# jdidion/atropos

Measured on AMD Instinct MI355X. Metric: reads/s (whole node) 150 bp SE adapter-align, higher is better.
Workload: dtype int32

## Files before the change

atropos_amd/csrc/filter_kernels.hip:

```cpp
#define ATR_DEFINE_FILTER_KERNELS
#include "locate_fast.hpp"
#include "side_stream.hpp"

namespace atr {

constexpr long long FAST_SERIAL_READS = 65536;
constexpr long long FAST_SERIAL_READS_LINKED = 64;

window_launcher window_group_0(int), window_group_1(int), window_group_2(int), window_group_3(int);

static BandParams band_params(const atr_aligner *a) {
    BandParams bp;
    memset(&bp, 0, sizeof(bp));
    for (int i = 0; i < a->p.m && i < FILTER_MAX_M; ++i) bp.rrep[i] = (uint32_t)(a->codes[i] & 15u) * 0x11111111u;
    bp.and_mode = (a->wildcard_ref || a->wildcard_query) ? 1 : 0;
    bp.noindel = a->indel_cost > a->p.k ? 1 : 0;
    return bp;
}

int launch_linked_band(const void *d_wave, int nad, bool and_mode, const uint4 *packed, const int32_t *lens, long long nreads,
                       int nchunks, int max_len, const uint4 *front, uint4 *out, FastWork wk, hipStream_t st);

static LinkedArgs no_linked_args() {
    LinkedArgs la;
    memset(&la, 0, sizeof(la));
    return la;
}

typedef window_launcher (*window_group_fn)(int);
static const window_group_fn window_groups[4] = {window_group_0, window_group_1, window_group_2, window_group_3};

void launch_fast_scan(FastWork wk, hipStream_t st) {
    hipLaunchKernelGGL(scan_bins_kernel, dim3((wk.nused + SCAN_CHUNK - 1) / SCAN_CHUNK, wk.nbins / 256), dim3(256), 0, st, wk);
    hipLaunchKernelGGL(scan_total_kernel, dim3(1), dim3(1024), 0, st, wk);
}

constexpr int DP_STREAMS = 4;
int launch_fast_dp(const atr_aligner *a, const uint4 *packed, const int32_t *lens, long long nreads, int nchunks,
                   int max_len, uint4 *out, FastWork wk, const LinkedArgs *la, int idx, int count, hipStream_t st, bool planes,
                   bool one_stream) {
    static thread_local SideStream side[DP_STREAMS];
    if (planes && la) return (int)hipErrorInvalidValue;
    if (count < 1 || count > DP_STREAMS || idx < 0 || idx >= count) return (int)hipErrorInvalidValue;
    hipError_t e = hipSuccess;
    const bool serial = one_stream || nreads <= (count == 1 ? FAST_SERIAL_READS : FAST_SERIAL_READS_LINKED);
    if (serial) {
        const BandParams bp = band_params(a);
        const dim3 bgrid((unsigned)std::max<long long>(1, std::min<long long>((nreads + 3) / 4, 4096)));
        const LinkedArgs none = la ? *la : no_linked_args();
        if (la) {
            if (bp.and_mode) hipLaunchKernelGGL((band_kernel<true, true>), bgrid, dim3(256), 0, st, a->p, bp, packed, lens, nreads, nchunks, max_len, out, wk, none);
            else             hipLaunchKernelGGL((band_kernel<false, true>), bgrid, dim3(256), 0, st, a->p, bp, packed, lens, nreads, nchunks, max_len, out, wk, none);
        } else if (planes) {
            if (bp.and_mode) hipLaunchKernelGGL((band_kernel<true, false, true>), bgrid, dim3(256), 0, st, a->p, bp, packed, lens, nreads, nchunks, max_len, out, wk, none);
            else             hipLaunchKernelGGL((band_kernel<false, false, true>), bgrid, dim3(256), 0, st, a->p, bp, packed, lens, nreads, nchunks, max_len, out, wk, none);
        } else {
            if (bp.and_mode) hipLaunchKernelGGL((band_kernel<true, false>), bgrid, dim3(256), 0, st, a->p, bp, packed, lens, nreads, nchunks, max_len, out, wk, none);
            else             hipLaunchKernelGGL((band_kernel<false, false>), bgrid, dim3(256), 0, st, a->p, bp, packed, lens, nreads, nchunks, max_len, out, wk, none);
        }
        e = hipGetLastError();
        if (e != hipSuccess) return (int)e;
        const int mts = round_up_rows(a->p.m) / ROW_GRAN - 1;
        return window_groups[mts / 4](mts % 4)(a, packed, lens, nreads, nchunks, max_len, out, wk, la, st, planes);
    }
    const int nside = (la && la->win_count != 1) ? 1 : std::min(count, 3);
    hipStream_t bst = st;
    if (idx == 0) {
        static const bool urgent = [] { const char *x = getenv("ATR_WINDOW_PRIORITY"); return !(x && x[0] == '0'); }();
        for (int k = 0; k < nside; ++k) if (!side[k].ready(urgent)) return (int)hipErrorInvalidValue;
        e = hipEventRecord(side[0].fork, st);
        for (int k = 0; k < nside && e == hipSuccess; ++k) e = hipStreamWaitEvent(side[k].stream, side[0].fork, 0);
        if (e != hipSuccess) return (int)e;
    }
    const dim3 block(256);
    {
        const BandParams bp = band_params(a);
        const dim3 bgrid((unsigned)std::min<long long>((nreads + 255) / 256, 4096));
        if (la && la->multi) {
            if (idx == 0) {
                const int rc = launch_linked_band(la->multi, count, la->multi_and, packed, lens, nreads, nchunks, max_len, la->front,
                                                  out, wk, bst);
                if (rc != 0) return rc;
            }
        } else if (la) {
            if (bp.and_mode) hipLaunchKernelGGL((band_kernel<true, true>), bgrid, block, 0, bst, a->p, bp, packed, lens, nreads, nchunks, max_len, out, wk, *la);
            else             hipLaunchKernelGGL((band_kernel<false, true>), bgrid, block, 0, bst, a->p, bp, packed, lens, nreads, nchunks, max_len, out, wk, *la);
        } else if (planes) {
            const LinkedArgs none = no_linked_args();
            if (bp.and_mode) hipLaunchKernelGGL((band_kernel<true, false, true>), bgrid, block, 0, bst, a->p, bp, packed, lens, nreads, nchunks, max_len, out, wk, none);
            else             hipLaunchKernelGGL((band_kernel<false, false, true>), bgrid, block, 0, bst, a->p, bp, packed, lens, nreads, nchunks, max_len, out, wk, none);
        } else {
            const LinkedArgs none = no_linked_args();
            if (bp.and_mode) hipLaunchKernelGGL((band_kernel<true, false>), bgrid, block, 0, bst, a->p, bp, packed, lens, nreads, nchunks, max_len, out, wk, none);
            else             hipLaunchKernelGGL((band_kernel<false, false>), bgrid, block, 0, bst, a->p, bp, packed, lens, nreads, nchunks, max_len, out, wk, none);
        }
    }
    e = hipGetLastError();
    if (e != hipSuccess) return (int)e;
    const int mt = round_up_rows(a->p.m) / ROW_GRAN - 1;
    const int rc = window_groups[mt / 4](mt % 4)(a, packed, lens, nreads, nchunks, max_len, out, wk, la,
                                                 side[idx % nside].stream, planes);
    if (rc != 0) return rc;
    if (idx == count - 1) {
        for (int k = 0; k < nside && e == hipSuccess; ++k) {
            e = hipEventRecord(side[k].join, side[k].stream);
            if (e == hipSuccess) e = hipStreamWaitEvent(st, side[k].join, 0);
        }
    }
    return (int)e;
}

int launch_locate_fast(const atr_aligner *a, const uint4 *packed, const int32_t *lens, long long nreads,
                       int nchunks, int max_len, uint4 *out, void *work, hipStream_t st) {
    FastWork wk = fast_carve(work, nreads);
    wk.nused = fast_blocks_for((nreads + 63) / 64);
    wk.lpw = nreads <= 8192 ? 0 : 64;
    const FilterParams &fp = aligner_filter_params(a);
    const bool wide = fp.rows > 32, ragged = lens != nullptr;
    const dim3 grid(wk.nused), block(256);
    if (wide) {
        if (ragged) hipLaunchKernelGGL((filter_kernel<true, true>), grid, block, 0, st, a->p, fp, packed, lens, nreads, nchunks, max_len, out, wk);
        else        hipLaunchKernelGGL((filter_kernel<true, false>), grid, block, 0, st, a->p, fp, packed, lens, nreads, nchunks, max_len, out, wk);
    } else {
        if (ragged) hipLaunchKernelGGL((filter_kernel<false, true>), grid, block, 0, st, a->p, fp, packed, lens, nreads, nchunks, max_len, out, wk);
        else        hipLaunchKernelGGL((filter_kernel<false, false>), grid, block, 0, st, a->p, fp, packed, lens, nreads, nchunks, max_len, out, wk);
    }
    launch_fast_scan(wk, st);
    hipLaunchKernelGGL(scatter_kernel, dim3(wk.nused), dim3(256), 0, st, nreads, a->p.m,
                       (!ragged || !(a->flags & ATR_START_WITHIN_SEQ1)) ? 1 : 0, wk);
    return launch_fast_dp(a, packed, lens, nreads, nchunks, max_len, out, wk, nullptr, 0, 1, st, false, false);
}

int launch_prefix_band(const atr_aligner *a, const uint4 *packed, const int32_t *lens, long long nreads, int nchunks,
                       int max_len, uint4 *out, hipStream_t st) {
    const BandParams bp = band_params(a);
    const dim3 grid((unsigned)((nreads + 255) / 256)), block(256);
    if (bp.and_mode) hipLaunchKernelGGL((prefix_band_kernel<true>), grid, block, 0, st, a->p, bp, packed, lens, nreads, nchunks, max_len, out);
    else             hipLaunchKernelGGL((prefix_band_kernel<false>), grid, block, 0, st, a->p, bp, packed, lens, nreads, nchunks, max_len, out);
    return (int)hipGetLastError();
}

}
```

atropos_amd/csrc/locate_fast.hpp:

```cpp
#ifndef ATR_LOCATE_FAST_HPP
#define ATR_LOCATE_FAST_HPP

#include <algorithm>
#include "locate_kernel.hpp"
#include "filter_core.hpp"
#include "linked_core.hpp"
#include "piece_core.hpp"
#include "fast_work.hpp"

namespace atr {
inline const FilterParams &aligner_filter_params(const atr_aligner *a) {
    struct Slot { unsigned long long uid = 0; FilterParams fp; };
    static thread_local Slot slots[4];
    static thread_local unsigned turn = 0;
    if (a->uid != 0)
        for (Slot &s : slots) if (s.uid == a->uid) return s.fp;
    Slot &s = slots[turn++ & 3u];
    s.fp = filter_params(a->peq, a->codes, a->p.m, a->flags, a->wildcard_ref || a->wildcard_query, a->p.thr, a->p.min_overlap);
    s.uid = a->uid;
    return s.fp;
}
inline const FilterParams &aligner_piece_filter_params(const atr_aligner *a) {
    struct Slot { unsigned long long uid = 0; FilterParams fp; };
    static thread_local Slot slots[4];
    static thread_local unsigned turn = 0;
    if (a->uid != 0)
        for (Slot &s : slots) if (s.uid == a->uid) return s.fp;
    Slot &s = slots[turn++ & 3u];
    s.fp = filter_params(a->peq, a->codes, a->p.m, a->flags, a->wildcard_ref || a->wildcard_query, a->p.thr, a->p.min_overlap, true);
    s.uid = a->uid;
    return s.fp;
}
}

namespace atr {

struct LinkedArgs {
    int bin0;
    const uint4 *front;
    LinkedPost post;
    const void *multi;
    bool multi_and;
    const LocateParams *multi_p;
    const LinkedPost *multi_post;
    int a0, win_count;
};

inline int fast_blocks_for(long long ntiles) {
    return (int)std::max<long long>(1, std::min<long long>(FAST_BLOCKS, (ntiles + 3) / 4));
}

__device__ __forceinline__ int dp_lanes_per_wave(long long tasks, long long grid_waves, int fixed) {
    if (fixed) return fixed;
    int lpw = 1;
    while (lpw < 64 && (long long)lpw * grid_waves < tasks) lpw <<= 1;
    return lpw;
}

constexpr int SCAN_CHUNK = 64, SCAN_CHUNKS = FAST_BLOCKS / SCAN_CHUNK;
static_assert(FAST_BLOCKS % SCAN_CHUNK == 0 && SCAN_CHUNKS % 16 == 0 && SCAN_CHUNK % 16 == 0, "scan kernels walk 16 rows at a time");
__device__ __forceinline__ uint32_t fast_slot0(const FastWork &wk, int bin) {
    return wk.binbase[bin] + wk.chunks[(size_t)(blockIdx.x / SCAN_CHUNK) * wk.nbins + bin] +
           wk.counts[(size_t)blockIdx.x * wk.nbins + bin];
}

#ifdef ATR_DEFINE_FILTER_KERNELS
template <bool WIDE, bool RAGGED>
__global__ __launch_bounds__(256) void filter_kernel(const LocateParams p, const FilterParams fp,
                                                     const uint4 *__restrict__ packed,
                                                     const int32_t *__restrict__ lens, long long nreads, int nchunks,
                                                     int max_len, uint4 *__restrict__ out, FastWork wk) {
    __shared__ uint2 s_peq[16];
    __shared__ uint32_t s_hist[FILTER_BINS];
    const Uniform u = make_uniform(p, round_up_rows_dev(p.m));
    if (threadIdx.x < 16) s_peq[threadIdx.x] = make_uint2((uint32_t)fp.peq[threadIdx.x], (uint32_t)(fp.peq[threadIdx.x] >> 32));
    if (threadIdx.x < FILTER_BINS) s_hist[threadIdx.x] = 0;
    __syncthreads();

    const int lane = threadIdx.x & 63, wave = __builtin_amdgcn_readfirstlane((int)(threadIdx.x >> 6));
    const long long ntiles = (nreads + 63) >> 6;
    long long t0, t1;
    block_tiles(ntiles, t0, t1, wk.nused);
    for (long long tile = t0 + wave; tile < t1; tile += 4) {
        const long long r = tile * 64 + lane;
        const bool live = r < nreads;
        const int n = live ? (RAGGED ? lens[r] : max_len) : 0;
        FilterState F;
        filter_init(F, u, fp.rows);
        const int jhi = RAGGED ? wave_max_i32(n) : max_len;
        const int jfull = RAGGED ? wave_min_i32(live ? n : 0x7fffffff) : max_len;
        const uint4 *tp = packed + (size_t)tile * nchunks * 64 + lane;
        if (jhi > 0) {
            const int c1 = (jhi + 31) >> 5;
            uint4 nxt = tp[0];
            uint2 ea[8], eb[8];
            auto fetch_masks = [&](uint32_t w, uint2 (&e)[8]) { fetch_peq8(s_peq, w, e); };
            const uint32_t kreg = (uint32_t)u.k;
            fetch_masks(nxt.x, ea);
            for (int c = 0; c < c1; ++c) {
                uint4 cur = nxt;
                if (c + 1 < c1) nxt = tp[(size_t)(c + 1) * 64];
                int j = c * 32;
#pragma unroll
                for (int d = 0; d < 4; ++d) {
                    uint2 (&e)[8] = (d & 1) ? eb : ea;
                    fetch_masks(d == 0 ? cur.y : d == 1 ? cur.z : d == 2 ? cur.w : nxt.x, (d & 1) ? ea : eb);
                    if (j + 8 <= (RAGGED ? jfull : jhi)) {
#pragma unroll
                        for (int b = 0; b < 8; ++b) filter_step<WIDE>(F, e[b].x, e[b].y, kreg);
                        j += 8;
                    } else {
#pragma unroll
                        for (int b = 0; b < 8; ++b) {
                            ++j;
                            if (j <= jhi && (!RAGGED || j <= n)) filter_step<WIDE>(F, e[b].x, e[b].y, kreg);
                        }
                    }
                    if (j >= jhi) break;
                }
                filter_fold(F, RAGGED ? min(n, min(j, jhi)) : min(j, jhi), fp.rows, kreg);
            }
        }
        uint32_t ww_lane = 0u;
        if (live) {
            uint32_t rec[4];
            const uint32_t ww = filter_decide<WIDE>(F, u, fp, (const uint32_t *)tp, nchunks, n, rec);
            ww_lane = ww;
            if (!window_valid(ww)) out[r] = make_uint4(rec[0], rec[1], rec[2], rec[3]);
            else atomicAdd(&s_hist[window_bin(ww, u.m, !RAGGED || ragged_rows_bins(u.sr))], 1u);
        }
        const uint64_t um = __ballot(window_valid(ww_lane));
        if (lane == 0) wk.mask[tile] = um;
        if (window_valid(ww_lane)) wk.win[tile * 64 + __popcll(um & ((1ull << lane) - 1ull))] = ww_lane;
    }
    __syncthreads();
    if (threadIdx.x < FILTER_BINS) wk.counts[(size_t)blockIdx.x * FILTER_BINS + threadIdx.x] = s_hist[threadIdx.x];
}

__global__ __launch_bounds__(256) void scan_bins_kernel(FastWork wk) {
    const int bin = blockIdx.y * 256 + threadIdx.x;
    uint32_t *col = wk.counts + (size_t)blockIdx.x * SCAN_CHUNK * wk.nbins + bin;
    const int rows = min(SCAN_CHUNK, wk.nused - (int)blockIdx.x * SCAN_CHUNK);
    uint32_t run = 0;
    for (int b0 = 0; b0 < rows; b0 += 16) {
        uint32_t v[16];
#pragma unroll
        for (int i = 0; i < 16; ++i) v[i] = b0 + i < rows ? col[(size_t)(b0 + i) * wk.nbins] : 0u;
#pragma unroll
        for (int i = 0; i < 16; ++i) { if (b0 + i < rows) col[(size_t)(b0 + i) * wk.nbins] = run; run += v[i]; }
    }
    wk.chunks[(size_t)blockIdx.x * wk.nbins + bin] = run;
}

__global__ __launch_bounds__(1024) void scan_total_kernel(FastWork wk) {
    __shared__ uint32_t s_part[1024];
    const int b = threadIdx.x;
    uint32_t mine = 0u;
    if (b < wk.nbins) {
        uint32_t *col = wk.chunks + b;
        const int chunks = (wk.nused + SCAN_CHUNK - 1) / SCAN_CHUNK;
        for (int c0 = 0; c0 < chunks; c0 += 16) {
            uint32_t v[16];
#pragma unroll
            for (int i = 0; i < 16; ++i) v[i] = c0 + i < chunks ? col[(size_t)(c0 + i) * wk.nbins] : 0u;
#pragma unroll
            for (int i = 0; i < 16; ++i) { if (c0 + i < chunks) col[(size_t)(c0 + i) * wk.nbins] = mine; mine += v[i]; }
        }
    }
    s_part[b] = mine;
    __syncthreads();
    for (int off = 1; off < 1024; off <<= 1) {
        const uint32_t add = b >= off ? s_part[b - off] : 0u;
        __syncthreads();
        s_part[b] += add;
        __syncthreads();
    }
    if (b < wk.nbins) wk.binbase[b] = s_part[b] - mine;
    if (b == 1023) { wk.binbase[wk.nbins] = s_part[1023]; wk.total[0] = s_part[1023]; }
}

__global__ __launch_bounds__(256) void scatter_kernel(long long nreads, int m, int by_rows, FastWork wk) {
    __shared__ uint32_t s_cur[FILTER_BINS];
    if (threadIdx.x < FILTER_BINS)
        s_cur[threadIdx.x] = fast_slot0(wk, threadIdx.x);
    __syncthreads();
    const long long ntiles = (nreads + 63) >> 6;
    long long t0, t1;
    block_tiles(ntiles, t0, t1, wk.nused);
    constexpr int SCATTER_ROUNDS = 4;
    const long long rend = min(nreads, t1 * 64);
    for (long long r0 = t0 * 64 + threadIdx.x; r0 < rend; r0 += 256 * SCATTER_ROUNDS) {
        uint64_t um[SCATTER_ROUNDS];
        uint32_t ww[SCATTER_ROUNDS];
#pragma unroll
        for (int t = 0; t < SCATTER_ROUNDS; ++t) {
            const long long r = r0 + 256 * t;
            um[t] = r < rend ? wk.mask[r >> 6] : 0ull;
        }
#pragma unroll
        for (int t = 0; t < SCATTER_ROUNDS; ++t) {
            const long long r = r0 + 256 * t;
            const int lane = (int)(r & 63);
            ww[t] = ((um[t] >> lane) & 1ull) ? wk.win[(r & ~63ll) + __popcll(um[t] & ((1ull << lane) - 1ull))] : 0u;
        }
#pragma unroll
        for (int t = 0; t < SCATTER_ROUNDS; ++t) {
            const long long r = r0 + 256 * t;
            if (window_valid(ww[t]))
                wk.order[atomicAdd(&s_cur[window_bin(ww[t], m, by_rows != 0)], 1u)] = make_uint2((uint32_t)r, ww[t]);
        }
    }
}
template <bool AND_MODE, bool LINKED, bool PLANES = false>
__global__ __launch_bounds__(256) void band_kernel(const LocateParams p, const BandParams bp,
                                                   const uint4 *__restrict__ packed, const int32_t *__restrict__ lens,
                                                   long long nreads, int nchunks, int max_len, uint4 *__restrict__ out,
                                                   FastWork wk, const LinkedArgs la) {
    __shared__ int16_t s_thr[ATR_MAX_REF_LEN + 2];
    __shared__ uint32_t s_stream[4][BAND_STREAM][64];
    __shared__ uint32_t s_spread_flat[PLANES ? 1024 : 1];
    uint32_t (*s_spread)[256] = (uint32_t (*)[256])s_spread_flat;
    const Uniform u = make_uniform(p, round_up_rows_dev(p.m));
    for (int i = threadIdx.x; i <= u.m + 1; i += 256) s_thr[i] = p.thr[i];
    if constexpr (PLANES) piece_spread_fill(s_spread);
    __syncthreads();
    const long long base = LINKED ? (long long)wk.binbase[la.bin0] : 0;
    const long long total = (long long)wk.binbase[(LINKED ? la.bin0 : 0) + BAND_BINS];
    const int lane = threadIdx.x & 63;
    const int lpw = dp_lanes_per_wave(total - base, (long long)gridDim.x * 4, wk.lpw);
    const long long nwaves = (total - base + lpw - 1) / lpw;
    for (long long wv = (long long)blockIdx.x * 4 + __builtin_amdgcn_readfirstlane((int)(threadIdx.x >> 6)); wv < nwaves;
         wv += (long long)gridDim.x * 4) {
        const long long slot = base + wv * lpw + lane;
        const bool live = lane < lpw && slot < total;
        const uint2 task = live ? wk.order[slot] : make_uint2(0u, 0u);
        const long long r = (long long)task.x;
        const uint32_t ww = task.y;
        const int n = live ? (lens ? lens[r] : max_len) : 0;
        const bool last = live && window_scan(ww);
        const bool any_last = wave_max_i32(last ? 1 : 0) != 0, any_rowm = wave_max_i32(live && !last ? 1 : 0) != 0;
        const int s_lane = (live && !last) ? window_hi(ww) - u.m + u.k - window_lo(ww) : 0;
        const int smax = min(BAND_W - 1, wave_max_i32(s_lane));
        const uint32_t *q = (const uint32_t *)(packed + ((size_t)(r >> 6) * nchunks) * 64 + (r & 63));
        uint32_t *ns = &s_stream[__builtin_amdgcn_readfirstlane((int)(threadIdx.x >> 6))][0][lane];
        if constexpr (PLANES) {
            const bool dense = live && (ww & PIECE_NODENSE) == 0u;
            if (dense) {
                const uint32_t di = wk.dref[slot];
                const uint4 a = wk.tdata[2 * (size_t)di], b = wk.tdata[2 * (size_t)di + 1];
                ns[0] = a.x; ns[64] = a.y; ns[128] = a.z; ns[192] = a.w;
                ns[256] = b.x; ns[320] = b.y; ns[384] = b.z; ns[448] = b.w;
            }
            if (wave_max_i32(live && !dense ? 1 : 0) != 0) {
                if (!dense) band_stage_planes(q, nchunks, window_lo(ww), ns, 64, s_spread, band_stream_dwords(u.m));
            }
        } else band_stage(q, nchunks, window_lo(ww), ns, 64, band_stream_dwords(u.m));
        uint32_t rec[4] = {0xFFFF0000u, 0u, 0u, 0u};
        if (any_rowm) band_locate<AND_MODE>(u, bp.rrep, bp.noindel != 0, ns, 64, n, ww, smax, s_thr, rec);
        if (any_last) {
            const int smax_l = min(BAND_W - 1, wave_max_i32(last ? last_band_width(ww) : 0));
            const int rows_max = wave_max_i32(last ? (last_band_rowm(ww) ? u.m : window_rows(ww)) : 0);
            const int cap_lo = wave_min_i32(last ? window_rows(ww) - last_band_span(ww) : 0x7fffffff);
            uint32_t rec_l[4];
            band_locate_last<AND_MODE>(u, bp.rrep, bp.noindel != 0, ns, 64, n, ww, last, smax_l, rows_max, cap_lo, s_thr, rec_l);
            if (last) { rec[0] = rec_l[0]; rec[1] = rec_l[1]; rec[2] = rec_l[2]; rec[3] = rec_l[3]; }
        }
        if (LINKED && live)
            linked_finish(rec, (int)(la.front[r].y >> 16), la.post.m, la.post.min_overlap, la.post.pf_thr,
                          la.post.accept_full != 0, la.post.rmp, la.post.rmp_ld, la.post.max_rmp);
        if (live) out[r] = make_uint4(rec[0], rec[1], rec[2], rec[3]);
    }
}
template <bool AND_MODE>
__global__ __launch_bounds__(256) void prefix_band_kernel(const LocateParams p, const BandParams bp,
                                                          const uint4 *__restrict__ packed,
                                                          const int32_t *__restrict__ lens, long long nreads,
                                                          int nchunks, int max_len, uint4 *__restrict__ out) {
    __shared__ int16_t s_thr[ATR_MAX_REF_LEN + 2];
    __shared__ uint32_t s_stream[4][BAND_STREAM][64];
    const Uniform u = make_uniform(p, round_up_rows_dev(p.m));
    for (int i = threadIdx.x; i <= u.m + 1; i += 256) s_thr[i] = p.thr[i];
    __syncthreads();
    const int lane = threadIdx.x & 63;
    const long long tile = (long long)blockIdx.x * 4 + __builtin_amdgcn_readfirstlane((int)(threadIdx.x >> 6));
    if (tile * 64 >= nreads) return;
    const long long r = tile * 64 + lane;
    const bool live = r < nreads;
    const int n = live ? (lens ? lens[r] : max_len) : 0;
    const uint32_t *q = (const uint32_t *)(packed + (size_t)tile * nchunks * 64 + lane);
    uint32_t *ns = &s_stream[__builtin_amdgcn_readfirstlane((int)(threadIdx.x >> 6))][0][lane];
    band_stage(q, nchunks, -u.k, ns, 64, band_stream_dwords(u.m));
    uint32_t rec[4];
    band_locate_prefix<AND_MODE>(u, bp.rrep, bp.noindel != 0, ns, 64, n, s_thr, rec);
    if (live) out[r] = make_uint4(rec[0], rec[1], rec[2], rec[3]);
}
#endif

template <bool LINKED>
__device__ __forceinline__ const LocateParams &window_params(const LocateParams &p_arg, const LinkedArgs &la, int ad) {
    if constexpr (LINKED) return la.multi_p[ad];
    else return p_arg;
}

template <int MT, bool NOINDEL, bool LINKED, bool PLANES = false>
__global__ __launch_bounds__(256) void window_kernel(const LocateParams p_arg, const uint4 *__restrict__ packed,
                                                     const int32_t *__restrict__ lens, long long nreads,
                                                     int nchunks, int max_len, uint4 *__restrict__ out, FastWork wk,
                                                     const LinkedArgs la) {
    __shared__ int16_t s_thr[ATR_MAX_REF_LEN + 2];
    __shared__ uint32_t s_init[ATR_MAX_REF_LEN + 1];
    __shared__ __attribute__((aligned(16))) uint32_t s_nm[16][4];
    __shared__ uint32_t s_spread_flat[PLANES ? 1024 : 1];
    uint32_t (*s_spread)[256] = (uint32_t (*)[256])s_spread_flat;
    const int ad = LINKED ? la.a0 + (int)blockIdx.y : 0;
    const LocateParams &p = window_params<LINKED>(p_arg, la, ad);
    const Uniform u = make_uniform(p, MT);
    if (threadIdx.x < 64) s_nm[threadIdx.x >> 2][threadIdx.x & 3] = p.nmask[threadIdx.x >> 2][threadIdx.x & 3];
    for (int i = threadIdx.x; i <= MT + 1; i += 256) {
        if (i <= u.m + 1) s_thr[i] = p.thr[i];
        if (i <= MT) s_init[i] = init_word(i - u.p0, 0, u.sr, u.sq, u.indel);
    }
    if constexpr (PLANES) piece_spread_fill(s_spread);
    __syncthreads();
    const int bin0 = LINKED ? ad * FILTER_BINS : 0;
    const long long first = (long long)wk.binbase[bin0 + BAND_BINS], total = (long long)wk.binbase[bin0 + FILTER_BINS];
    const int lane = threadIdx.x & 63;
    const int lpw = dp_lanes_per_wave(total - first, (long long)gridDim.x * 4, wk.lpw);
    const long long nwaves = (total - first + lpw - 1) / lpw;
    for (long long wv = (long long)blockIdx.x * 4 + __builtin_amdgcn_readfirstlane((int)(threadIdx.x >> 6)); wv < nwaves;
         wv += (long long)gridDim.x * 4) {
        const long long slot = first + wv * lpw + lane;
        const bool live = lane < lpw && slot < total;
        const uint2 task = live ? wk.order[slot] : make_uint2(0u, 0u);
        const long long r = (long long)task.x;
        const uint32_t ww = task.y;
        const int n = live ? (lens ? lens[r] : max_len) : 0;
        const int j_lo = window_lo(ww), j_hi = live ? window_hi(ww) : 0;
        const bool has_window = live && j_hi > j_lo;
        const int jlo = wave_min_i32(live ? j_lo : 0x7fffffff);
        const int jhi = wave_max_i32(has_window ? j_hi : 0);
        const int rows_w = wave_max_i32(live ? window_rows(ww) : 0);
        const int plimit = u.p0 + rows_w;
        const bool head = !(u.sr && jlo == 0);
        const bool tri = __builtin_amdgcn_readfirstlane((int)(first + wv * lpw >= (long long)wk.binbase[bin0 + ROWS_BIN0])) != 0 &&
                         head && lens == nullptr;
        const int s_lane = (LINKED && live) ? (int)(la.front[r].y >> 16) : 0;
        const int s_top = LINKED ? wave_max_i32(s_lane) : 0;

        LaneState<MT> L;
        const uint4 *tp = packed + ((size_t)(r >> 6) * nchunks) * 64 + (r & 63);

        const bool rows_wave = __builtin_amdgcn_readfirstlane((int)(first + wv * lpw >= (long long)wk.binbase[bin0 + ROWS_BIN0])) != 0;
        if (!LINKED && lens != nullptr && rows_wave && !u.sr) {
            const int shift = live ? max_len - n : 0;
            const int v0 = wave_min_i32(live ? j_lo + shift : 0x7fffffff);
            if (max_len - v0 <= TAIL_COLUMNS && v0 < max_len) {
                const int s_top_t = wave_max_i32(shift);
                lane_init_window<MT, NOINDEL>(L, u, max_len, v0, live ? max_len : 0, live && window_scan(ww), s_init, s_thr);
                uint32_t tb[TAIL_COLUMNS / 8];
                {
                    const int dlo = n - TAIL_COLUMNS;
                    const int z0 = dlo >> 3;
                    const uint32_t sh = 4u * (uint32_t)(dlo & 7);
                    uint32_t raw[TAIL_COLUMNS / 8 + 1];
#pragma unroll
                    for (int t = 0; t <= TAIL_COLUMNS / 8; ++t) {
                        if constexpr (PLANES) raw[t] = live ? read_dword_planes((const uint32_t *)tp, nchunks, z0 + t, s_spread) : 0u;
                        else raw[t] = live ? read_dword((const uint32_t *)tp, nchunks, z0 + t) : 0u;
                    }
#pragma unroll
                    for (int t = 0; t < TAIL_COLUMNS / 8; ++t) tb[t] = sh ? ((raw[t] >> sh) | (raw[t + 1] << (32u - sh))) : raw[t];
                }
                int j = max_len - TAIL_COLUMNS;
#pragma unroll 1
                for (int d = 0; d < TAIL_COLUMNS / 8; ++d) {
                    uint32_t w = tb[0];
#pragma unroll
                    for (int t = 0; t + 1 < TAIL_COLUMNS / 8; ++t) tb[t] = tb[t + 1];
#pragma unroll 1
                    for (int b = 0; b < 8; ++b) {
                        ++j;
                        const uint32_t q = w & 15u;
                        w >>= 4;
                        if (j <= v0) continue;
                        uint32_t nm[(MT + 31) / 32];
                        load_mask(nm, s_nm, q);
                        int pl = min(plimit, u.p0 + (j - v0) + u.k);
                        pl = min(pl, u.p0 + triangle_rows(rows_w, max_len, j, u.k));
                        lane_step<MT, NOINDEL, true, true>(L, u, j, nm, s_thr, pl);
                        if (j <= s_top_t && shift == j) lane_restart_window<MT>(L, u, j);
                    }
                }
                if (live) {
                    uint32_t rec[4];
                    lane_result<MT>(L, u, rec);
                    if ((rec[0] >> 16) != 0xFFFFu) rec[1] -= (uint32_t)shift * 0x00010001u;
                    out[r] = make_uint4(rec[0], rec[1], rec[2], rec[3]);
                }
                continue;
            }
        }
        lane_init_window<MT, NOINDEL>(L, u, n, jlo, j_hi, live && window_scan(ww), s_init, s_thr);
        if (jhi > jlo) {
            const int c0 = jlo >> 5, c1 = (jhi + 31) >> 5;
            uint4 nxt = tp[(size_t)c0 * 64];
            for (int c = c0; c < c1; ++c) {
                uint4 cur = nxt;
                if (c + 1 < c1) nxt = tp[(size_t)(c + 1) * 64];
                if constexpr (PLANES) cur = make_uint4(piece_nibbles(s_spread, cur.x, cur.y, cur.z, cur.w, 0), piece_nibbles(s_spread, cur.x, cur.y, cur.z, cur.w, 1),
                                             piece_nibbles(s_spread, cur.x, cur.y, cur.z, cur.w, 2), piece_nibbles(s_spread, cur.x, cur.y, cur.z, cur.w, 3));
                int j = c * 32;
#pragma unroll 1
                for (int d = 0; d < 4; ++d) {
                    uint32_t w = cur.x;
                    cur.x = cur.y; cur.y = cur.z; cur.z = cur.w;
#pragma unroll 1
                    for (int b = 0; b < 8; ++b) {
                        ++j;
                        const uint32_t q = w & 15u;
                        w >>= 4;
                        if (j <= jlo || j > jhi) continue;
                        uint32_t nm[(MT + 31) / 32];
                        load_mask(nm, s_nm, q);
                        int pl = head ? min(plimit, u.p0 + (j - jlo) + u.k) : plimit;
                        if (tri) pl = min(pl, u.p0 + triangle_rows(rows_w, max_len, j, u.k));
                        lane_step<MT, NOINDEL, true, true>(L, u, j, nm, s_thr, pl);
                        if (LINKED && j <= s_top && s_lane == j) lane_restart_window<MT>(L, u, j);
                    }
                }
            }
        }
        if (live) {
            uint32_t rec[4];
            lane_result<MT>(L, u, rec);
            if constexpr (LINKED) {
                const LinkedPost &post = la.multi_post[ad];
                linked_finish(rec, s_lane, post.m, post.min_overlap, post.pf_thr, post.accept_full != 0,
                              post.rmp, post.rmp_ld, post.max_rmp);
            }
            out[r] = make_uint4(rec[0], rec[1], rec[2], rec[3]);
        }
    }
}

typedef int (*window_launcher)(const atr_aligner *, const uint4 *, const int32_t *, long long, int, int, uint4 *,
                               FastWork, const LinkedArgs *, hipStream_t, bool);

template <int MT>
int launch_window_mt(const atr_aligner *a, const uint4 *packed, const int32_t *lens, long long nreads, int nchunks,
                     int max_len, uint4 *out, FastWork wk, const LinkedArgs *la, hipStream_t st, bool planes) {
    const bool noindel = a->indel_cost > a->p.k;
    const dim3 grid((unsigned)std::max<long long>(1, std::min<long long>((nreads + 3) / 4, 4096))), block(256);
    if (la) {
        if (la->win_count < 1) return 0;
        const dim3 lgrid(grid.x, (unsigned)la->win_count);
        if (noindel) hipLaunchKernelGGL((window_kernel<MT, true, true>), lgrid, block, 0, st, a->p, packed, lens, nreads, nchunks, max_len, out, wk, *la);
        else         hipLaunchKernelGGL((window_kernel<MT, false, true>), lgrid, block, 0, st, a->p, packed, lens, nreads, nchunks, max_len, out, wk, *la);
    } else if (planes) {
        LinkedArgs none;
        memset(&none, 0, sizeof(none));
        if (noindel) hipLaunchKernelGGL((window_kernel<MT, true, false, true>), grid, block, 0, st, a->p, packed, lens, nreads, nchunks, max_len, out, wk, none);
        else         hipLaunchKernelGGL((window_kernel<MT, false, false, true>), grid, block, 0, st, a->p, packed, lens, nreads, nchunks, max_len, out, wk, none);
    } else {
        LinkedArgs none;
        memset(&none, 0, sizeof(none));
        if (noindel) hipLaunchKernelGGL((window_kernel<MT, true, false>), grid, block, 0, st, a->p, packed, lens, nreads, nchunks, max_len, out, wk, none);
        else         hipLaunchKernelGGL((window_kernel<MT, false, false>), grid, block, 0, st, a->p, packed, lens, nreads, nchunks, max_len, out, wk, none);
    }
    return (int)hipGetLastError();
}

constexpr int WINDOW_SIZES = FILTER_MAX_M / ROW_GRAN;

}
#endif
```

Before: 21.28 billion.

## Add persistent software-pipelined band kernel and decouple window lane packing from grid

```diff
diff --git a/atropos_amd/csrc/filter_kernels.hip b/atropos_amd/csrc/filter_kernels.hip
--- a/atropos_amd/csrc/filter_kernels.hip
+++ b/atropos_amd/csrc/filter_kernels.hip
@@ -27,6 +27,28 @@
     return la;
 }
 
+static bool band_planes_on() { const char *x = getenv("ATR_BAND_PERSIST"); return !(x && x[0] == '0'); }
+template <bool AND_MODE>
+static int band_planes_blocks(long long want) {
+    static thread_local int cached_dev = -1, cached = 0;
+    static const int forced = [] { const char *x = getenv("ATR_BAND_BLOCKS"); const int n = x ? atoi(x) : 0; return n >= 1 && n <= 65536 ? n : 0; }();
+    int dev = 0;
+    if (hipGetDevice(&dev) != hipSuccess) return (int)std::max<long long>(1, std::min<long long>(want, 1024));
+    if (dev != cached_dev) {
+        int per_cu = 0, cus = 0;
+        if (hipOccupancyMaxActiveBlocksPerMultiprocessor(&per_cu, band_planes_kernel<AND_MODE>, 256, 0) != hipSuccess || per_cu < 1) per_cu = 4;
+        if (hipDeviceGetAttribute(&cus, hipDeviceAttributeMultiprocessorCount, dev) != hipSuccess || cus < 1) cus = 256;
+        cached = per_cu * cus;
+        cached_dev = dev;
+    }
+    return (int)std::max<long long>(1, std::min<long long>(want, forced ? forced : cached));
+}
+static void launch_band_planes(const atr_aligner *a, const BandParams &bp, const uint4 *packed, const int32_t *lens, int nchunks,
+                               int max_len, uint4 *out, const FastWork &wk, long long want, hipStream_t st) {
+    if (bp.and_mode) hipLaunchKernelGGL((band_planes_kernel<true>), dim3(band_planes_blocks<true>(want)), dim3(256), 0, st, a->p, bp, packed, lens, nchunks, max_len, out, wk);
+    else             hipLaunchKernelGGL((band_planes_kernel<false>), dim3(band_planes_blocks<false>(want)), dim3(256), 0, st, a->p, bp, packed, lens, nchunks, max_len, out, wk);
+}
+
 typedef window_launcher (*window_group_fn)(int);
 static const window_group_fn window_groups[4] = {window_group_0, window_group_1, window_group_2, window_group_3};
 
@@ -51,6 +73,8 @@
         if (la) {
             if (bp.and_mode) hipLaunchKernelGGL((band_kernel<true, true>), bgrid, dim3(256), 0, st, a->p, bp, packed, lens, nreads, nchunks, max_len, out, wk, none);
             else             hipLaunchKernelGGL((band_kernel<false, true>), bgrid, dim3(256), 0, st, a->p, bp, packed, lens, nreads, nchunks, max_len, out, wk, none);
+        } else if (planes && band_planes_on()) {
+            launch_band_planes(a, bp, packed, lens, nchunks, max_len, out, wk, bgrid.x, st);
         } else if (planes) {
             if (bp.and_mode) hipLaunchKernelGGL((band_kernel<true, false, true>), bgrid, dim3(256), 0, st, a->p, bp, packed, lens, nreads, nchunks, max_len, out, wk, none);
             else             hipLaunchKernelGGL((band_kernel<false, false, true>), bgrid, dim3(256), 0, st, a->p, bp, packed, lens, nreads, nchunks, max_len, out, wk, none);
@@ -85,6 +109,8 @@
         } else if (la) {
             if (bp.and_mode) hipLaunchKernelGGL((band_kernel<true, true>), bgrid, block, 0, bst, a->p, bp, packed, lens, nreads, nchunks, max_len, out, wk, *la);
             else             hipLaunchKernelGGL((band_kernel<false, true>), bgrid, block, 0, bst, a->p, bp, packed, lens, nreads, nchunks, max_len, out, wk, *la);
+        } else if (planes && band_planes_on()) {
+            launch_band_planes(a, bp, packed, lens, nchunks, max_len, out, wk, bgrid.x, bst);
         } else if (planes) {
             const LinkedArgs none = no_linked_args();
             if (bp.and_mode) hipLaunchKernelGGL((band_kernel<true, false, true>), bgrid, block, 0, bst, a->p, bp, packed, lens, nreads, nchunks, max_len, out, wk, none);
diff --git a/atropos_amd/csrc/locate_fast.hpp b/atropos_amd/csrc/locate_fast.hpp
--- a/atropos_amd/csrc/locate_fast.hpp
+++ b/atropos_amd/csrc/locate_fast.hpp
@@ -272,6 +272,96 @@
     }
 }
 template <bool AND_MODE>
+__global__ __launch_bounds__(256) void band_planes_kernel(const LocateParams p, const BandParams bp,
+                                                          const uint4 *__restrict__ packed, const int32_t *__restrict__ lens,
+                                                          int nchunks, int max_len, uint4 *__restrict__ out, FastWork wk) {
+    __shared__ int16_t s_thr[ATR_MAX_REF_LEN + 2];
+    __shared__ uint32_t s_stream[4][BAND_STREAM][64];
+    __shared__ uint32_t s_spread_flat[1024];
+    uint32_t (*s_spread)[256] = (uint32_t (*)[256])s_spread_flat;
+    const Uniform u = make_uniform(p, round_up_rows_dev(p.m));
+    for (int i = threadIdx.x; i <= u.m + 1; i += 256) s_thr[i] = p.thr[i];
+    __syncthreads();
+    const long long total = (long long)wk.binbase[BAND_BINS];
+    const int lane = threadIdx.x & 63, wave = __builtin_amdgcn_readfirstlane((int)(threadIdx.x >> 6));
+    const long long stride = (long long)gridDim.x * 4;
+    const int lpw = dp_lanes_per_wave(total, stride, wk.lpw);
+    const long long nwaves = (total + lpw - 1) / lpw;
+    uint32_t *ns = &s_stream[wave][0][lane];
+    bool have_spread = false;
+
+    struct Task { uint2 e; uint32_t di; };
+    struct Rec { uint4 a, b; int n; };
+    const auto live_of = [&](long long wv) { return wv < nwaves && lane < lpw && wv * lpw + lane < total; };
+    const auto fetch_task = [&](long long wv, Task &t) {
+        const bool live = live_of(wv);
+        const long long slot = wv * lpw + lane;
+        t.e = live ? wk.order[slot] : make_uint2(0u, 0u);
+        t.di = live ? wk.dref[slot] : 0u;
+    };
+    const auto fetch_rec = [&](long long wv, const Task &t, Rec &r) {
+        const bool live = live_of(wv);
+        const bool dense = live && (t.e.y & PIECE_NODENSE) == 0u;
+        r.a = dense ? wk.tdata[2 * (size_t)t.di] : make_uint4(0u, 0u, 0u, 0u);
+        r.b = dense ? wk.tdata[2 * (size_t)t.di + 1] : make_uint4(0u, 0u, 0u, 0u);
+        r.n = live ? (lens ? lens[t.e.x] : max_len) : 0;
+    };
+    long long wv = (long long)blockIdx.x * 4 + wave;
+    Task t_cur, t_nxt;
+    Rec r_cur;
+    fetch_task(wv, t_cur);
+    fetch_task(wv + stride, t_nxt);
+    fetch_rec(wv, t_cur, r_cur);
+    for (; wv < nwaves; wv += stride) {
+        Rec r_nxt;
+        Task t_nn;
+        fetch_rec(wv + stride, t_nxt, r_nxt);
+        fetch_task(wv + 2 * stride, t_nn);
+
+        const bool live = live_of(wv);
+        const long long r = (long long)t_cur.e.x;
+        const uint32_t ww = t_cur.e.y;
+        const int n = r_cur.n;
+        const bool last = live && window_scan(ww);
+        const bool any_last = wave_max_i32(last ? 1 : 0) != 0, any_rowm = wave_max_i32(live && !last ? 1 : 0) != 0;
+        const int s_lane = (live && !last) ? window_hi(ww) - u.m + u.k - window_lo(ww) : 0;
+        const int smax = min(BAND_W - 1, wave_max_i32(s_lane));
+        const bool dense = live && (ww & PIECE_NODENSE) == 0u;
+        if (dense) {
+            ns[0] = r_cur.a.x; ns[64] = r_cur.a.y; ns[128] = r_cur.a.z; ns[192] = r_cur.a.w;
+            ns[256] = r_cur.b.x; ns[320] = r_cur.b.y; ns[384] = r_cur.b.z; ns[448] = r_cur.b.w;
+        }
+        if (wave_max_i32(live && !dense ? 1 : 0) != 0) {
+            if (!have_spread) {
+                for (int i = lane; i < 1024; i += 64) {
+                    const int t = i >> 8, b = i & 255;
+                    uint32_t v = 0;
+#pragma unroll
+                    for (int k = 0; k < 8; ++k) v |= (uint32_t)((b >> k) & 1) << (4 * k + t);
+                    s_spread[t][b] = v;
+                }
+                have_spread = true;
+            }
+            if (live && !dense) {
+                const uint32_t *q = (const uint32_t *)(packed + ((size_t)(r >> 6) * nchunks) * 64 + (r & 63));
+                band_stage_planes(q, nchunks, window_lo(ww), ns, 64, s_spread, band_stream_dwords(u.m));
+            }
+        }
+        uint32_t rec[4] = {0xFFFF0000u, 0u, 0u, 0u};
+        if (any_rowm) band_locate<AND_MODE>(u, bp.rrep, bp.noindel != 0, ns, 64, n, ww, smax, s_thr, rec);
+        if (any_last) {
+            const int smax_l = min(BAND_W - 1, wave_max_i32(last ? last_band_width(ww) : 0));
+            const int rows_max = wave_max_i32(last ? (last_band_rowm(ww) ? u.m : window_rows(ww)) : 0);
+            const int cap_lo = wave_min_i32(last ? window_rows(ww) - last_band_span(ww) : 0x7fffffff);
+            uint32_t rec_l[4];
+            band_locate_last<AND_MODE>(u, bp.rrep, bp.noindel != 0, ns, 64, n, ww, last, smax_l, rows_max, cap_lo, s_thr, rec_l);
+            if (last) { rec[0] = rec_l[0]; rec[1] = rec_l[1]; rec[2] = rec_l[2]; rec[3] = rec_l[3]; }
+        }
+        if (live) out[r] = make_uint4(rec[0], rec[1], rec[2], rec[3]);
+        t_cur = t_nxt; t_nxt = t_nn; r_cur = r_nxt;
+    }
+}
+template <bool AND_MODE>
 __global__ __launch_bounds__(256) void prefix_band_kernel(const LocateParams p, const BandParams bp,
                                                           const uint4 *__restrict__ packed,
                                                           const int32_t *__restrict__ lens, long long nreads,
@@ -325,7 +415,8 @@
     const int bin0 = LINKED ? ad * FILTER_BINS : 0;
     const long long first = (long long)wk.binbase[bin0 + BAND_BINS], total = (long long)wk.binbase[bin0 + FILTER_BINS];
     const int lane = threadIdx.x & 63;
-    const int lpw = dp_lanes_per_wave(total - first, (long long)gridDim.x * 4, wk.lpw);
+    const int lpw = wk.lpw < 0 ? dp_lanes_per_wave(total - first, (long long)-wk.lpw, 0)
+                               : dp_lanes_per_wave(total - first, (long long)gridDim.x * 4, wk.lpw);
     const long long nwaves = (total - first + lpw - 1) / lpw;
     for (long long wv = (long long)blockIdx.x * 4 + __builtin_amdgcn_readfirstlane((int)(threadIdx.x >> 6)); wv < nwaves;
          wv += (long long)gridDim.x * 4) {
@@ -443,6 +534,13 @@
     }
 }
 
+constexpr int WINDOW_LONG_WAVES = 2048;
+inline int window_long_waves() {
+    const char *x = getenv("ATR_WINDOW_WAVES");
+    const int n = x && *x ? atoi(x) : -1;
+    return n >= 0 && n <= 65536 ? n : WINDOW_LONG_WAVES;
+}
+
 typedef int (*window_launcher)(const atr_aligner *, const uint4 *, const int32_t *, long long, int, int, uint4 *,
                                FastWork, const LinkedArgs *, hipStream_t, bool);
 
@@ -459,6 +557,8 @@
     } else if (planes) {
         LinkedArgs none;
         memset(&none, 0, sizeof(none));
+        const int wwaves = window_long_waves();
+        if (wk.lpw == 64 && wwaves > 0) wk.lpw = -wwaves;
         if (noindel) hipLaunchKernelGGL((window_kernel<MT, true, false, true>), grid, block, 0, st, a->p, packed, lens, nreads, nchunks, max_len, out, wk, none);
         else         hipLaunchKernelGGL((window_kernel<MT, false, false, true>), grid, block, 0, st, a->p, packed, lens, nreads, nchunks, max_len, out, wk, none);
     } else {
```

New measurement: 20.26 billion. 0.952x the previous value.
